# bostoncleek/ergodic_exploration

Hardware: NVIDIA B200
Metric: ergodic control solves/sec (batched) (higher is better)
Workload: dtype f64

## Files before the change

ergodic_exploration_b200/csrc/ergodic_b200.cu:

```cuda
#include "../../include/ergodic_b200.h"

#include <cuda_runtime.h>

#include <algorithm>
#include <atomic>
#include <cmath>
#include <cstdio>
#include <cstdlib>
#include <cstring>
#include <new>
#include <string>
#include <vector>

#include <nvtx3/nvToolsExt.h>

#include "collision_kernels.cuh"
#include "map_target.cuh"
#include "map_target_batch.cuh"
#include "model_kernels.cuh"
#include "peer_gather.cuh"
#include "phik_dmma.cuh"
#include "phik_kernels.cuh"
#include "phik_tma.cuh"
#include "safe_control.cuh"
// ... 299 lines not shown
  cudaFree(p->d_ys);
  cudaFree(p->d_cx);
  cudaFree(p->d_cy);
  cudaFree(p->d_cxp);
  cudaFree(p->d_cxpf);
  cudaFree(p->d_cxt);
  cudaFree(p->d_cxtf);
  cudaFree(p->d_T);
  cudaFree(p->d_parts);
  cudaFree(p->d_phik);
  cudaFree(p->d_sum);
  cudaFree(p->d_phi_stage);
  cudaFree(p->d_done);
  for (double* q : p->w_cxt) cudaFree(q);
  for (double* q : p->w_cxtf) cudaFree(q);
  for (double* q : p->w_cy) cudaFree(q);
  cudaFree(p->d_wraw);
  delete p;
}

eb_status eb_phik_plan_set_stream(eb_phik_plan* p, void* s)
{
  if (!p) return fail(EB_ERR_INVALID_ARGUMENT, "plan is NULL");
  p->stream = static_cast<cudaStream_t>(s);
  return EB_OK;
}

eb_status eb_phik_plan_set_algo(eb_phik_plan* p, int algo)
{
  if (!p) return fail(EB_ERR_INVALID_ARGUMENT, "plan is NULL");
  if (algo < 0 || algo > 5)
    return fail(EB_ERR_INVALID_ARGUMENT, "algo must be 0 (auto), 1 (simple), 2 / 3 (register-streamed DMMA tiles, with / without "
                                         "the mirror fold) or 4 / 5 (TMA-staged DMMA tiles, with / without the mirror fold)");
  if (algo >= 2 && p->nb > 32)
    return fail(EB_ERR_UNSUPPORTED, "num_basis > 32: algo 0 (auto: the TMA tile kernel per block of 32 x 32 orders on large grids, "
                                    "else the simple pair) or 1 (simple pair)");
  if ((algo == 2 || algo == 3) && !eb::phik_dmma_supported(p->nx, p->ny))
    return fail(EB_ERR_UNSUPPORTED, "the register-streamed DMMA phi_k kernel needs nx % 4 == 0 and nx >= 128");
  if (algo >= 4 && (!eb::phik_tma_supported(p->nx, p->ny) || !eb::phik_tma_encoder()))
    return fail(EB_ERR_UNSUPPORTED, "the TMA phi_k kernel needs an even nx >= 64 and a driver with cuTensorMapEncodeTiled");
  p->algo = algo;
  return EB_OK;
}

long long eb_phik_launch_count(const eb_phik_plan* p) { return p ? p->launches : 0; }

eb_status eb_phik_plan_fold(const eb_phik_plan* p, int* fold, double* deviation)
{
  if (!p) return fail(EB_ERR_INVALID_ARGUMENT, "plan is NULL");
  if (fold) *fold = p->fold ? 1 : 0;
  if (deviation) *deviation = p->fold_dev;
  return EB_OK;
}

static eb_status phik_execute(eb_phik_plan* p, const double* phi_dev, double* phik_dev, double* phi_sum_dev,
                              double* raw_dev);

eb_status eb_phik_execute_dev(eb_phik_plan* p, const double* phi_dev, double* phik_dev, double* phi_sum_dev)
{
  if (!p || !phi_dev || !phik_dev) return fail(EB_ERR_INVALID_ARGUMENT, "eb_phik_execute_dev: NULL argument");
  return phik_execute(p, phi_dev, phik_dev, phi_sum_dev, nullptr);
}

eb_status eb_phik_execute_raw_dev(eb_phik_plan* p, const double* phi_dev, double* raw_dev)
{
  if (!p || !phi_dev || !raw_dev) return fail(EB_ERR_INVALID_ARGUMENT, "eb_phik_execute_raw_dev: NULL argument");
  return phik_execute(p, phi_dev, nullptr, nullptr, raw_dev);
}

static eb_status phik_execute(eb_phik_plan* p, const double* phi_dev, double* phik_dev, double* phi_sum_dev,
                              double* raw_dev)
{
  EB_TRACE("eb_phik_execute");
  EB_CUDA(cudaSetDevice(p->device));
  int algo = p->algo;
  if (p->nb > 32 && p->d_wraw && algo != 1 && (reinterpret_cast<uintptr_t>(phi_dev) & 15) == 0)
  {
    const int ld = p->ld, nblk = ld / 32;
    for (int by = 0; by < nblk; by++)
      for (int bx = 0; bx < nblk; bx++)
      {
        const int nbm = std::min(32, p->nb - 32 * std::min(by, bx));
        const eb::PhikTmaOut out{ p->d_done, nbm, nullptr, nullptr, p->d_wraw + 1024 * ((size_t)by * nblk + bx), nullptr };
        const int np = eb::phik_tma_launch(phi_dev, p->nx, p->ny, p->fold ? p->w_cxtf[bx] : p->w_cxt[bx], p->w_cy[by],
                                           p->d_parts, p->max_parts, p->fold, out, p->stream);
        if (np < 0) return fail(EB_ERR_CUDA, std::string("phik_tma_launch (wide): ") + cudaGetErrorString(cudaGetLastError()));
        p->launches += 1;
      }
    eb::phik_assemble_wide<<<(ld * ld + 255) / 256, 256, 0, p->stream>>>(p->d_wraw, p->nb, nblk, ld, phik_dev, phi_sum_dev, raw_dev);
    p->launches += 1;
    EB_CUDA(cudaGetLastError());
    return EB_OK;
  }
  if (p->nb > 32)
  {
    const int ld = p->ld;
    eb::phik_stage1_simple<<<dim3(p->ny, ld / 32), 256, 0, p->stream>>>(phi_dev, p->nx, p->d_cx, ld, p->d_T);
    eb::phik_stage2_simple<<<dim3(p->nb, ld / 32), 256, 0, p->stream>>>(p->d_T, p->ny, p->d_cy, ld, p->d_parts);
    eb::phik_finalize_wide<<<(ld * ld + 255) / 256, 256, 0, p->stream>>>(p->d_parts, p->nb, ld, phik_dev, phi_sum_dev, raw_dev);
    p->launches += 3;
    EB_CUDA(cudaGetLastError());
    return EB_OK;
  }
  const bool big = (long long)p->nx * p->ny >= (1 << 18);
  if (algo == 0)
    algo = (big && eb::phik_tma_supported(p->nx, p->ny) && eb::phik_tma_encoder() && (reinterpret_cast<uintptr_t>(phi_dev) & 15) == 0) ? 4 :
           (big && eb::phik_dmma_supported(p->nx, p->ny))                                                                        ? 2 :
                                                                                                                                   1;
  int nparts = 1;
  const bool fold = (algo == 2 || algo == 4) && p->fold;
  if (algo >= 4)
  {
    const eb::PhikTmaOut out{ p->d_done, p->nb, phik_dev, phi_sum_dev, raw_dev, p->peer };
    nparts = eb::phik_tma_launch(phi_dev, p->nx, p->ny, fold ? p->d_cxtf : p->d_cxt, p->d_cy, p->d_parts, p->max_parts, fold,
                                 out, p->stream);
    if (nparts < 0) return fail(EB_ERR_CUDA, std::string("phik_tma_launch: ") + cudaGetErrorString(cudaGetLastError()));
    p->launches += 1;
    return EB_OK;
  }
  else if (algo >= 2)
  {
    nparts = eb::phik_dmma_launch(phi_dev, p->nx, p->ny, fold ? p->d_cxpf : p->d_cxp, p->d_cy, p->d_parts, p->max_parts,
                                  fold, p->stream);
    if (nparts < 0) return fail(EB_ERR_CUDA, std::string("phik_dmma_launch: ") + cudaGetErrorString(cudaGetLastError()));
    p->launches += 1;
  }
  else
  {
    eb::phik_stage1_simple<<<p->ny, 256, 0, p->stream>>>(phi_dev, p->nx, p->d_cx, eb::kPhikLd, p->d_T);
    eb::phik_stage2_simple<<<32, 256, 0, p->stream>>>(p->d_T, p->ny, p->d_cy, eb::kPhikLd, p->d_parts);
    p->launches += 2;
  }
  eb::phik_finalize<<<1, 1024, 0, p->stream>>>(p->d_parts, nparts, p->nb, fold ? 1 : 0, phik_dev, phi_sum_dev, raw_dev);
  p->launches += 1;
  EB_CUDA(cudaGetLastError());
  return EB_OK;
}

eb_status eb_phik_execute_host(eb_phik_plan* p, const double* phi, double* phik, double* phi_sum)
{
  EB_TRACE("eb_phik_execute_host");
  if (!p || !phi || !phik) return fail(EB_ERR_INVALID_ARGUMENT, "eb_phik_execute_host: NULL argument");
  EB_CUDA(cudaSetDevice(p->device));
  const size_t bytes = sizeof(double) * (size_t)p->nx * p->ny;
  if (!p->d_phi_stage) EB_CUDA(cudaMalloc(&p->d_phi_stage, bytes));
  double* const d_phi = p->d_phi_stage;
  cudaError_t e = cudaMemcpyAsync(d_phi, phi, bytes, cudaMemcpyHostToDevice, p->stream);
  eb_status st = EB_OK;
  if (e == cudaSuccess) st = eb_phik_execute_dev(p, d_phi, p->d_phik, p->d_sum);
  if (e == cudaSuccess && st == EB_OK)
    e = cudaMemcpyAsync(phik, p->d_phik, sizeof(double) * p->nb * p->nb, cudaMemcpyDeviceToHost, p->stream);
  if (e == cudaSuccess && st == EB_OK && phi_sum)
    e = cudaMemcpyAsync(phi_sum, p->d_sum, sizeof(double), cudaMemcpyDeviceToHost, p->stream);
  if (e == cudaSuccess && st == EB_OK) e = cudaStreamSynchronize(p->stream);
  if (st != EB_OK) return st;
  if (e != cudaSuccess) return fail(EB_ERR_CUDA, std::string("eb_phik_execute_host: ") + cudaGetErrorString(e));
  return EB_OK;
}

eb_status eb_phik_from_grid_host(int device, const double* phi, int nx, int ny, double resolution, double lx,
                                 double ly, int nb, double* phik, double* phi_sum)
{
  eb_phik_plan* p = nullptr;
  eb_status st = eb_phik_plan_create(device, nx, ny, resolution, lx, ly, nb, &p);
  if (st != EB_OK) return st;
  st = eb_phik_execute_host(p, phi, phik, phi_sum);
  eb_phik_plan_destroy(p);
  return st;
}

}

struct PeerLaunch
{
  int n_peer = 0;
  double* u0_peer[eb::kMaxPeers] = {};
  unsigned long long* flag_peer[eb::kMaxPeers] = {};
  unsigned long long flag_value = 0;
  unsigned int* done_counter = nullptr;
  const unsigned long long* my_flags = nullptr;
  unsigned long long need = 0;
};

struct eb_controller
{
  eb_config cfg{};
  int N = 0, K = 0, nb = 0, B = 0;
  cudaStream_t stream = nullptr;
  double* d_ut[2] = { nullptr, nullptr };
  int cur = 0;
  double* d_pose = nullptr;
  double* d_hist = nullptr;
  double* d_hist_cos = nullptr;
  long long cos_count = 0;
  double cos_key[4] = { 0.0, 0.0, 0.0, 0.0 };
  long long hist_cap = 0, mem_count = 0;
  double *d_phik = nullptr, *d_lamk = nullptr;
  double *d_u0 = nullptr, *d_metric = nullptr, *d_ck = nullptr, *d_x = nullptr;
  double* d_xt = nullptr;
  double* d_big_scratch = nullptr;
  int big_rows = 0;
  int *d_mem_idx_in = nullptr, *d_mem_idx_out = nullptr;
  int *h_fault = nullptr, *d_fault = nullptr;
  int last_idx_count = 0;
  double lx = 0.0, ly = 0.0;
  double map_pos[2] = { 0.0, 0.0 };
  std::vector<double> gauss_mu, gauss_sigma;
  eb_phik_plan* plan = nullptr;
  double* d_phi_grid = nullptr;
  size_t phi_grid_cells = 0;
  double* d_gauss = nullptr;
  int gauss_cap = 0;
  unsigned long long call = 0;
  long long launches = 0;
  bool have_pose = false;
  bool keep_ck = true;
  const struct PeerLaunch* peer = nullptr;
  bool per_inst = false;
  bool frames_set = false;
  double* d_phik_b = nullptr;
  double* d_frames = nullptr;
  double *d_gmu = nullptr, *d_gsig = nullptr;
  int* d_gcount = nullptr;
  int gmax = 0;
  double* d_bounds = nullptr;
  eb::MapBatchDesc* h_mb_desc = nullptr;
  eb::MapBatchDesc* d_mb_desc = nullptr;
  cudaEvent_t mb_staged = nullptr;
  double* d_mb_slots = nullptr;
  long long mb_slot_units = 0;
  unsigned* d_mb_arrive = nullptr;
  signed char* h_mb_cells = nullptr;
  signed char* d_mb_cells = nullptr;
  size_t mb_cells_bytes = 0;
  int mb_grid = 0;
  struct KeptKey
  {
    unsigned long long grid = 0, map = 0;
    unsigned nx = 0, ny = 0;
    double res = 0.0;
  };
  double* d_kb = nullptr;
  std::vector<int> kb_slot0, kb_cap;
  std::vector<KeptKey> kb_key;
  eb::MapKept* h_mb_kept = nullptr;
  eb::MapKept* d_mb_kept = nullptr;
  int* d_safe_list = nullptr;
  int* d_safe_branch = nullptr;
  double* d_safe_vb = nullptr;
  int safe_grid = 0;

  static double* mapped(const void* host)
  {
    cudaPointerAttributes a{};
    if (cudaPointerGetAttributes(&a, host) != cudaSuccess)
    {
      cudaGetLastError();
      return nullptr;
    }
    return (a.type == cudaMemoryTypeHost && a.devicePointer) ? static_cast<double*>(a.devicePointer) : nullptr;
  }
};

inline int zero_copy_max_batch()
{
  static const int v = [] {
    const char* e = std::getenv("EB_ZEROCOPY_MAX_BATCH");
    return e ? std::atoi(e) : 16384;
  }();
  return v;
}

inline bool replay_cos_cache()
{
  static const bool v = [] {
    const char* e = std::getenv("EB_REPLAY_COS");
    return !e || std::atoi(e) != 0;
  }();
  return v;
}

namespace
{
template <int MODEL, int NB, bool V2, bool PER_INST = false>
struct SolveLaunch
{
  static constexpr int kWide = []() constexpr {
    if constexpr (V2)
      return eb::Solve2Cfg<NB>::kWideWarps;
    else
      return eb::SolveCfg<NB>::kWideWarps;
  }();
  static size_t smem(int N, int warps = eb::kSolveWarps)
  {
    if constexpr (V2)
      return eb::solve2_smem_bytes<NB>(N, warps);
    else
      return eb::solve_smem_bytes(eb::SolveCfg<NB>::kTabDoubles, eb::SolveCfg<NB>::kFields, (N + 31) / 32, warps);
  }
  template <int WARPS>
  static cudaError_t launch_w(const eb::SolveParams& p, cudaStream_t s)
  {
    const size_t bytes = smem(p.N, WARPS);
    static size_t configured[64] = {};
    int dev = 0;
    cudaGetDevice(&dev);
    auto kernel = [] {
      if constexpr (V2)
        return eb::solve_kernel2<MODEL, NB, WARPS, PER_INST>;
      else
        return eb::solve_kernel<MODEL, NB, WARPS, PER_INST>;
    }();
    if (bytes > configured[dev & 63])
    {
      cudaError_t e = cudaFuncSetAttribute(kernel, cudaFuncAttributeMaxDynamicSharedMemorySize, (int)bytes);
      if (e != cudaSuccess) return e;
      configured[dev & 63] = bytes;
    }
    const int grid = (p.B + WARPS - 1) / WARPS;
    cudaLaunchConfig_t cfg = {};
    cfg.gridDim = dim3((unsigned)grid);
    cfg.blockDim = dim3((unsigned)(WARPS * 32));
    cfg.dynamicSmemBytes = bytes;
    cfg.stream = s;
    cudaLaunchAttribute at[1];
    at[0].id = cudaLaunchAttributeProgrammaticStreamSerialization;
    at[0].val.programmaticStreamSerializationAllowed = 1;
    cfg.attrs = at;
    cfg.numAttrs = 1;
    return cudaLaunchKernelEx(&cfg, kernel, p);
  }
  static cudaError_t launch(const eb::SolveParams& p, cudaStream_t s)
  {
    static const int sms = [] {
      int dev = 0, n = 148;
      cudaGetDevice(&dev);
      cudaDeviceGetAttribute(&n, cudaDevAttrMultiProcessorCount, dev);
      return n;
    }();
    static const bool wide_ok = [] {
      const char* e = std::getenv("EB_SOLVE_WIDE");
      return !e || std::atoi(e) != 0;
    }();
    if (wide_ok && p.n_peer == 0 && p.B <= sms * kWide && p.B > sms * eb::kSolveWarps && smem(p.N, kWide) + 2048 <= wide_limit())
      return launch_w<kWide>(p, s);
    return launch_w<eb::kSolveWarps>(p, s);
  }
  static size_t wide_limit()
  {
    static const size_t lim = [] {
      int dev = 0, v = 0;
      cudaGetDevice(&dev);
      cudaDeviceGetAttribute(&v, cudaDevAttrMaxSharedMemoryPerBlockOptin, dev);
      return (size_t)v;
    }();
    return lim;
  }
};

template <int MODEL, bool PER_INST>
cudaError_t launch_solve_big(const eb::SolveParams& p, cudaStream_t s)
{
  const size_t bytes = eb::solve_big_smem_bytes(p.nb, p.N);
  static size_t configured[64] = {};
  int dev = 0;
  cudaGetDevice(&dev);
  if (bytes > configured[dev & 63])
  {
    cudaError_t e = cudaFuncSetAttribute(eb::solve_kernel_big<MODEL, PER_INST>, cudaFuncAttributeMaxDynamicSharedMemorySize, (int)bytes);
    if (e != cudaSuccess) return e;
    configured[dev & 63] = bytes;
  }
  if (!p.big_scratch || p.big_rows < 1) return cudaErrorInvalidValue;
  const int grid = std::min(p.B, p.big_rows);
  eb::solve_kernel_big<MODEL, PER_INST><<<grid, eb::kBigThreads, bytes, s>>>(p, p.big_scratch);
  return cudaGetLastError();
}

int solve_big_resident(int nb, int N)
{
  const size_t bytes = eb::solve_big_smem_bytes(nb, N);
  int dev = 0, sms = 148, per_sm = 0;
  cudaGetDevice(&dev);
  cudaDeviceGetAttribute(&sms, cudaDevAttrMultiProcessorCount, dev);
  if (cudaFuncSetAttribute(eb::solve_kernel_big<0>, cudaFuncAttributeMaxDynamicSharedMemorySize, (int)bytes) != cudaSuccess ||
      cudaOccupancyMaxActiveBlocksPerMultiprocessor(&per_sm, eb::solve_kernel_big<0>, eb::kBigThreads, bytes) != cudaSuccess)
  {
    cudaGetLastError();
    per_sm = 1;
  }
  return sms * std::max(1, per_sm);
}

template <int MODEL, bool PER_INST, class F>
auto with_solve_launch(int nb, F&& f)
{
  if (nb <= 8) return f(SolveLaunch<MODEL, 8, false, PER_INST>{});
  if (nb <= 10) return f(SolveLaunch<MODEL, 10, false, PER_INST>{});
  if (nb <= 12) return f(SolveLaunch<MODEL, 12, false, PER_INST>{});
  if (nb <= 16) return f(SolveLaunch<MODEL, 16, true, PER_INST>{});
  if (nb <= 20) return f(SolveLaunch<MODEL, 20, true, PER_INST>{});
  if (nb <= 24) return f(SolveLaunch<MODEL, 24, true, PER_INST>{});
  return f(SolveLaunch<MODEL, 32, false, PER_INST>{});
}

template <int MODEL, bool PER_INST>
cudaError_t launch_solve_m(const eb::SolveParams& p, cudaStream_t s)
{
  if (p.nb > 32) return launch_solve_big<MODEL, PER_INST>(p, s);
  return with_solve_launch<MODEL, PER_INST>(p.nb, [&](auto L) { return decltype(L)::launch(p, s); });
}

size_t solve_smem_for(int nb, int N)
{
  if (nb > 32) return eb::solve_big_smem_bytes(nb, N);
  return with_solve_launch<0, false>(nb, [&](auto L) { return decltype(L)::smem(N); });
}

cudaError_t launch_solve(const eb::SolveParams& p, int model, cudaStream_t s, bool per_inst)
{
  if (per_inst)
    return model == EB_MODEL_OMNI ? launch_solve_m<eb::kModelOmni, true>(p, s) :
                                    launch_solve_m<eb::kModelSimpleCart, true>(p, s);
  return model == EB_MODEL_OMNI ? launch_solve_m<eb::kModelOmni, false>(p, s) :
                                  launch_solve_m<eb::kModelSimpleCart, false>(p, s);
}

eb_status ensure_hist(eb_controller* c, long long need)
{
  if (need <= c->hist_cap) return EB_OK;
  long long cap = std::max<long long>(c->hist_cap ? 2 * c->hist_cap : 128, need);
  {
    size_t free_b = 0, total_b = 0;
    const size_t full = sizeof(double) * (replay_cos_cache() ? 5 : 3) * (size_t)c->B * (size_t)c->cfg.buffer_size;
    if (cudaMemGetInfo(&free_b, &total_b) == cudaSuccess && full <= free_b / 8) cap = std::max<long long>(cap, c->cfg.buffer_size);
  }
  cap = std::min<long long>(cap, std::max<long long>((long long)c->cfg.buffer_size, need));
  double* nh = nullptr;
  EB_CUDA(cudaMalloc(&nh, sizeof(double) * 3 * (size_t)c->B * (size_t)cap));
  if (c->mem_count > 0)
    EB_CUDA(cudaMemcpyAsync(nh, c->d_hist, sizeof(double) * 3 * (size_t)c->B * (size_t)c->mem_count,
                            cudaMemcpyDeviceToDevice, c->stream));
  EB_CUDA(cudaStreamSynchronize(c->stream));
  cudaFree(c->d_hist);
  c->d_hist = nh;
  c->hist_cap = cap;
  if (replay_cos_cache() && c->per_inst)
  {
    double* nc = nullptr;
    EB_CUDA(cudaMalloc(&nc, sizeof(double) * 2 * (size_t)c->B * (size_t)cap));
    if (c->mem_count > 0 && c->d_hist_cos)
    {
      EB_CUDA(cudaMemcpyAsync(nc, c->d_hist_cos, sizeof(double) * 2 * (size_t)c->B * (size_t)c->mem_count,
                              cudaMemcpyDeviceToDevice, c->stream));
      EB_CUDA(cudaStreamSynchronize(c->stream));
    }
    cudaFree(c->d_hist_cos);
    c->d_hist_cos = nc;
  }
  else if (replay_cos_cache())
  {
    cudaFree(c->d_hist_cos);
    c->d_hist_cos = nullptr;
    c->cos_count = 0;
    EB_CUDA(cudaMalloc(&c->d_hist_cos, sizeof(double) * 2 * (size_t)c->B * (size_t)cap));
  }
  return EB_OK;
}

eb_status ensure_hist_cos(eb_controller* c)
{
  if (!c->d_hist_cos || c->mem_count == 0) return EB_OK;
  const double key[4] = { c->map_pos[0], c->map_pos[1], 1.0 / c->lx, 1.0 / c->ly };
  if (std::memcmp(key, c->cos_key, sizeof(key)) != 0)
  {
    std::memcpy(c->cos_key, key, sizeof(key));
    c->cos_count = 0;
  }
  if (c->cos_count < c->mem_count)
  {
    const long long n = (c->mem_count - c->cos_count) * (long long)c->B;
    const size_t off = (size_t)c->cos_count * (size_t)c->B;
    eb::hist_cos_kernel<<<(unsigned)((n + 255) / 256), 256, 0, c->stream>>>(c->d_hist + 3 * off, c->d_hist_cos + 2 * off, n,
                                                                            key[0], key[1], key[2], key[3]);
    EB_CUDA(cudaGetLastError());
    c->launches += 1;
    c->cos_count = c->mem_count;
  }
  return EB_OK;
}

eb_status check_fault(eb_controller* c)
{
  EB_CUDA(cudaStreamSynchronize(c->stream));
  const int f = *static_cast<volatile int*>(c->h_fault);
  if (f)
  {
    *c->h_fault = 0;
    if (f & 2)
      return fail(EB_ERR_OUT_OF_RANGE, "replay-buffer sample index outside [0, stored states)");
    if (f & 4) return fail(EB_ERR_CUDA, "control(): non-finite state or control signal (NaN / Inf guard)");
    if (f & eb::kFaultTarget)
      return fail(EB_ERR_INVALID_ARGUMENT, "per-instance target: an instance's map extent changed but it has no "
                                           "Gaussians (eb_set_target_gaussians_batch), or its extent is not positive");
    return fail(EB_ERR_INVALID_ARGUMENT, "Invalid twist y-velocity must be 0.");
  }
  return EB_OK;
}

eb_status refuse_per_inst(const char* call)
{
  return fail(EB_ERR_INVALID_ARGUMENT, std::string(call) + ": the controller holds one target per instance (it has "
                                                           "taken an eb_*_batch target call); use the _batch calls");
}

eb_status ensure_per_inst(eb_controller* c)
{
  if (c->per_inst) return EB_OK;
  EB_CUDA(cudaSetDevice(c->cfg.device));
  const size_t pb = sizeof(double) * (size_t)c->K * c->B, fb = sizeof(double) * eb::kFrDoubles * (size_t)c->B;
  EB_CUDA(cudaMalloc(&c->d_phik_b, pb));
  EB_CUDA(cudaMalloc(&c->d_frames, fb));
  EB_CUDA(cudaMalloc(&c->d_gcount, sizeof(int) * (size_t)c->B));
  EB_CUDA(cudaMalloc(&c->d_bounds, sizeof(double) * 4 * (size_t)c->B));
  EB_CUDA(cudaMemsetAsync(c->d_phik_b, 0, pb, c->stream));
  EB_CUDA(cudaMemsetAsync(c->d_frames, 0, fb, c->stream));
  EB_CUDA(cudaMemsetAsync(c->d_gcount, 0, sizeof(int) * (size_t)c->B, c->stream));
  c->per_inst = true;
  return EB_OK;
}

eb_status target_batch(eb_controller* c, const double* bounds_dev, const double* extent_dev, int* rebuilt_dev)
{
  eb::TargetBatchParams tp{};
  tp.B = c->B;
  tp.nb = c->nb;
  tp.max_n = c->gmax;
  tp.res = c->cfg.resolution;
  tp.bounds = bounds_dev;
  tp.extent = extent_dev;
  tp.counts = c->d_gcount;
  tp.mu = c->d_gmu;
  tp.sigma = c->d_gsig;
  tp.frames = c->d_frames;
  tp.phik = c->d_phik_b;
  tp.rebuilt = rebuilt_dev;
  tp.hist = c->d_hist;
  tp.hist_cos = c->d_hist_cos;
  tp.mem_count = c->d_hist_cos ? c->mem_count : 0;
  tp.fault = c->d_fault;
  eb::target_batch_kernel<<<c->B, eb::kTbThreads, sizeof(double) * 6 * (size_t)c->gmax, c->stream>>>(tp);
  EB_CUDA(cudaGetLastError());
  c->launches += 1;
  c->frames_set = true;
  return EB_OK;
}
}

extern "C" {

eb_status eb_create(const eb_config* cfg, eb_controller** out)
{
  if (!out) return fail(EB_ERR_INVALID_ARGUMENT, "eb_create: out is NULL");
  *out = nullptr;
  if (!cfg) return fail(EB_ERR_INVALID_ARGUMENT, "eb_create: cfg is NULL");
  if (cfg->model != EB_MODEL_SIMPLE_CART && cfg->model != EB_MODEL_OMNI)
    return fail(EB_ERR_INVALID_ARGUMENT, "eb_create: unknown model (only the 3-twist models SimpleCart and Omni "
                                         "can be driven by ErgodicControl)");
  if (cfg->batch < 1) return fail(EB_ERR_INVALID_ARGUMENT, "eb_create: batch must be >= 1");
  if (cfg->num_basis < 1 || cfg->num_basis > EB_MAX_NUM_BASIS)
    return fail(EB_ERR_INVALID_ARGUMENT, "eb_create: num_basis must be in 1.." + std::to_string(EB_MAX_NUM_BASIS));
  if (!(cfg->dt != 0.0) || !std::isfinite(cfg->horizon / cfg->dt))
    return fail(EB_ERR_INVALID_ARGUMENT, "eb_create: dt must be non-zero and finite");
  const unsigned steps = static_cast<unsigned>(std::abs(cfg->horizon / cfg->dt));
  if (steps == 1)
    return fail(EB_ERR_INVALID_ARGUMENT,
                "Need at least two steps in forward simulation. Increase the horizon or decrease the time step.");
  if (steps == 0) return fail(EB_ERR_INVALID_ARGUMENT, "eb_create: horizon / dt gives zero steps");
  if (steps > 4096) return fail(EB_ERR_UNSUPPORTED, "eb_create: more than 4096 horizon steps is not supported");
  if (eb_device_count() < 1) return fail(EB_ERR_NO_DEVICE, "no CUDA device is visible; there is no CPU fallback");
  EB_CUDA(cudaSetDevice(cfg->device));
  {
    int optin = 0;
    EB_CUDA(cudaDeviceGetAttribute(&optin, cudaDevAttrMaxSharedMemoryPerBlockOptin, cfg->device));
    const size_t need = solve_smem_for(static_cast<int>(cfg->num_basis), static_cast<int>(steps));
    if (need > static_cast<size_t>(optin))
      return fail(EB_ERR_UNSUPPORTED, "eb_create: a horizon of " + std::to_string(steps) + " steps with num_basis " +
                                          std::to_string(cfg->num_basis) + " needs " + std::to_string(need) +
                                          " bytes of shared memory per block; the device allows " + std::to_string(optin));
  }

  eb_controller* c = new (std::nothrow) eb_controller();
  if (!c) return fail(EB_ERR_CUDA, "out of host memory");
  c->cfg = *cfg;
  c->N = (int)steps;
  c->nb = (int)cfg->num_basis;
  c->K = c->nb * c->nb;
  c->B = cfg->batch;
  const size_t utb = sizeof(double) * 3 * (size_t)c->N * c->B;
  auto cleanup = [&](eb_status st) {
    eb_destroy(c);
    return st;
  };
#define EB_CUDA_C(expr)                                                                      \
  do                                                                                         \
  {                                                                                          \
    cudaError_t e__ = (expr);                                                                \
    if (e__ != cudaSuccess)                                                                  \
      return cleanup(fail(EB_ERR_CUDA, std::string(#expr) + ": " + cudaGetErrorString(e__))); \
  } while (0)
  EB_CUDA_C(cudaMalloc(&c->d_ut[0], utb));
  EB_CUDA_C(cudaMalloc(&c->d_ut[1], utb));
  EB_CUDA_C(cudaMemset(c->d_ut[0], 0, utb));
  EB_CUDA_C(cudaMemset(c->d_ut[1], 0, utb));
  EB_CUDA_C(cudaMalloc(&c->d_pose, sizeof(double) * 3 * c->B));
  EB_CUDA_C(cudaMemset(c->d_pose, 0, sizeof(double) * 3 * c->B));
  EB_CUDA_C(cudaMalloc(&c->d_x, sizeof(double) * 3 * c->B));
  EB_CUDA_C(cudaMalloc(&c->d_u0, sizeof(double) * 3 * c->B));
  EB_CUDA_C(cudaMalloc(&c->d_metric, sizeof(double) * c->B));
  EB_CUDA_C(cudaMalloc(&c->d_ck, sizeof(double) * (size_t)c->K * c->B));
// ... 3310 lines not shown
```

ergodic_exploration_b200/csrc/solve_kernel.cuh:

```cuda
#pragma once

#include "common.cuh"

namespace eb
{
constexpr int kModelSimpleCart = 0;
constexpr int kModelOmni = 1;
constexpr int kSolveWarps = 4;
constexpr int kMaxPeers = 8;
constexpr int kPeerBuffers = 4;
constexpr int kTabSlots = 16;
constexpr int kTabStride = 20;

#ifdef EB_PHASE_TIMING
constexpr int kPhaseSlots = 16;
__device__ long long g_phase[65536 * kPhaseSlots];
#define EB_PHASE(idx)                                                                      \
  do                                                                                       \
  {                                                                                        \
    if (lane == 0 && inst < 65536) g_phase[inst * kPhaseSlots + (idx)] = clock64();        \
  } while (0)
#else
#define EB_PHASE(idx) do { } while (0)
#endif

#ifdef EB_DEBUG_DUMP
__device__ double g_dbg[4096 * 16];
#endif

#ifndef EB_ABL
#define EB_ABL 0
#endif
__device__ __forceinline__ void abl_xor(double& d0, double a, double b)
{
  d0 = __hiloint2double(__double2hiint(d0), __double2loint(d0) ^ __double2loint(a) ^ __double2hiint(b));
}
__device__ __forceinline__ void dmma_ck(double& d0, double& d1, double a, double b)
{
#if EB_ABL & 1
  abl_xor(d0, a, b);
#else
  dmma884(d0, d1, a, b);
#endif
}
__device__ __forceinline__ void dmma_gr(double& d0, double& d1, double a, double b)
{
#if EB_ABL & 2
  abl_xor(d0, a, b);
#else
  dmma884(d0, d1, a, b);
#endif
}

struct SolveParams
{
  int B, N, M, nb;
  int mem_count, batch_size, idx_mode;
  double dt, lx, ly, inv_lx, inv_ly, ax, by, xmin, ymin, w;
  double Rinv[9], umin[3], umax[3], bw, beps;
  unsigned long long seed, call;
  const double* x;
  double* pose_out;
  const double* ut_in;
  double* ut_out;
  const double* hist;
  const double* hist_cos;
  const int* mem_idx;
  int* mem_idx_out;
  const double* phik;
  const double* lamk;
  double* u0;
  double* metric;
  double* ck;
  int* fault;
  int n_peer;
  double* u0_peer[kMaxPeers];
  unsigned long long* flag_peer[kMaxPeers];
  unsigned long long flag_value;
  unsigned int* done_counter;
  const unsigned long long* my_flags;
  unsigned long long need;
  double* big_scratch;
  int big_rows;
  const double* frames;
};

enum FrameField
{
  kFrXmin,
  kFrYmin,
  kFrLx,
  kFrLy,
  kFrInvLx,
  kFrInvLy,
  kFrAx,
  kFrBy,
  kFrDoubles
};

template <bool PER_INST, int F>
__device__ __forceinline__ double frame(const SolveParams& p, const int inst)
{
  if constexpr (PER_INST)
    return __ldg(p.frames + (size_t)inst * kFrDoubles + F);
  else if constexpr (F == kFrXmin)
    return p.xmin;
  else if constexpr (F == kFrYmin)
    return p.ymin;
  else if constexpr (F == kFrLx)
    return p.lx;
  else if constexpr (F == kFrLy)
    return p.ly;
  else if constexpr (F == kFrInvLx)
    return p.inv_lx;
  else if constexpr (F == kFrInvLy)
    return p.inv_ly;
  else if constexpr (F == kFrAx)
    return p.ax;
  else
    return p.by;
}

template <bool PER_INST>
__device__ __forceinline__ double phik_at(const SolveParams& p, const int inst, const int K, const int k)
{
  if constexpr (PER_INST)
    return __ldg(p.phik + (size_t)inst * K + k);
  else
    return __ldg(p.phik + k);
}

__device__ __forceinline__ void publish_first_twist(const SolveParams& p, const int inst, const int lane, const double (&un)[3])
{
  const double a0 = __shfl_sync(kFull, un[0], 0), a1 = __shfl_sync(kFull, un[1], 0), a2 = __shfl_sync(kFull, un[2], 0);
  const double mine = lane == 0 ? a0 : (lane == 1 ? a1 : a2);
  if (lane < 3) p.u0[(size_t)inst * 3 + lane] = mine;
  if (p.n_peer > 0)
  {
    if (lane < p.n_peer)
      while (*(const volatile unsigned long long*)(p.my_flags + lane) < p.need) __nanosleep(100);
    __syncwarp();
    if (lane < 3)
    {
#pragma unroll
      for (int q = 0; q < kMaxPeers; q++)
        if (q < p.n_peer) p.u0_peer[q][(size_t)inst * 3 + lane] = mine;
    }
    __threadfence();
    __syncwarp();
    if (lane == 0)
    {
      const unsigned int prev = atomicAdd(p.done_counter, 1u);
      if (prev == (unsigned int)p.B - 1u)
      {
        *p.done_counter = 0u;
        __threadfence_system();
#pragma unroll
        for (int q = 0; q < kMaxPeers; q++)
          if (q < p.n_peer) *(volatile unsigned long long*)p.flag_peer[q] = p.flag_value;
      }
    }
  }
}

template <int WARPS>
struct WideIo
{
  static constexpr bool kOn = WARPS > kSolveWarps;
  double x[kOn ? 3 * WARPS : 1];
  double u0[kOn ? 3 * WARPS : 1];
  unsigned int arrived;
};

template <int WARPS>
__device__ __forceinline__ void wide_io_load(WideIo<WARPS>& io, const SolveParams& p)
{
  const int first = blockIdx.x * WARPS;
  const int cnt = min(WARPS, p.B - first);
  if ((int)threadIdx.x < 3 * cnt) io.x[threadIdx.x] = p.x[(size_t)first * 3 + threadIdx.x];
  if (threadIdx.x == 0) io.arrived = 0u;
  __syncthreads();
}

template <int WARPS>
__device__ __forceinline__ void wide_io_store(WideIo<WARPS>& io, const SolveParams& p, const int lane, const int warp,
                                              const double (&un)[3])
{
  const double a0 = __shfl_sync(kFull, un[0], 0), a1 = __shfl_sync(kFull, un[1], 0), a2 = __shfl_sync(kFull, un[2], 0);
  if (lane < 3) io.u0[3 * warp + lane] = lane == 0 ? a0 : (lane == 1 ? a1 : a2);
  const int first = blockIdx.x * WARPS;
  const int cnt = min(WARPS, p.B - first);
  __syncwarp();
  unsigned int last = 0u;
  if (lane == 0)
  {
    __threadfence_block();
    last = atomicAdd(&io.arrived, 1u) == (unsigned int)(cnt - 1) ? 1u : 0u;
    __threadfence_block();
  }
  if (__shfl_sync(kFull, last, 0))
    for (int i = lane; i < 3 * cnt; i += 32) p.u0[(size_t)first * 3 + i] = io.u0[i];
}

__device__ __forceinline__ void grid_dependency_wait()
{
  asm volatile("griddepcontrol.wait;" ::: "memory");
  asm volatile("griddepcontrol.launch_dependents;" ::: "memory");
}

template <int MODEL>
__device__ __forceinline__ void model_f(double u0, double u1, double c, double s, double& fx, double& fy)
{
  if (MODEL == kModelOmni)
  {
    fx = u0 * c - u1 * s;
    fy = u0 * s + u1 * c;
  }
  else
  {
    fx = u0 * c;
    fy = u0 * s;
  }
}

struct RolloutCarry
{
  double x, y, th, cth, sth;
};

template <int MODEL>
__device__ __forceinline__ void rollout_round(const double dt, const bool valid, const int lane, const double u0,
                                              const double u1, const double u2, RolloutCarry& cy, double& xo,
                                              double& yo, double& tho, double& ce, double& se)
{
  const double dth = valid ? (dt / 6.0) * (((u2 + 2.0 * u2) + 2.0 * u2) + u2) : 0.0;
  const double inc = warp_scan_incl(dth, lane);
  double exc = __shfl_up_sync(kFull, inc, 1);
  if (lane == 0) exc = 0.0;
  const double th_before = cy.th + exc;
  tho = cy.th + inc;
  const double thm = th_before + dt * (0.5 * u2);
  double sm, cm;
  fast_sincos(tho, &se, &ce);
  fast_sincos(thm, &sm, &cm);
  double cb = __shfl_up_sync(kFull, ce, 1), sb = __shfl_up_sync(kFull, se, 1);
  if (lane == 0)
  {
    cb = cy.cth;
    sb = cy.sth;
  }
  double k1x, k1y, k2x, k2y, k4x, k4y;
  model_f<MODEL>(u0, u1, cb, sb, k1x, k1y);
  model_f<MODEL>(u0, u1, cm, sm, k2x, k2y);
  model_f<MODEL>(u0, u1, ce, se, k4x, k4y);
  const double dx = valid ? (dt / 6.0) * (((k1x + 2.0 * k2x) + 2.0 * k2x) + k4x) : 0.0;
  const double dy = valid ? (dt / 6.0) * (((k1y + 2.0 * k2y) + 2.0 * k2y) + k4y) : 0.0;
  xo = cy.x + warp_scan_incl(dx, lane);
  yo = cy.y + warp_scan_incl(dy, lane);
  cy.x = __shfl_sync(kFull, xo, 31);
  cy.y = __shfl_sync(kFull, yo, 31);
  cy.th = __shfl_sync(kFull, tho, 31);
  cy.cth = __shfl_sync(kFull, ce, 31);
  cy.sth = __shfl_sync(kFull, se, 31);
}

template <int NB>
__device__ __forceinline__ void coeff_chunk(double* __restrict__ tabx, const int lane, const bool valid,
                                            const int nvalid, const double c1x, const double c1y,
                                            double (&acc)[(NB + 7) / 8][(NB + 7) / 8][2])
{
  constexpr int TILES = (NB + 7) / 8;
  static_assert(NB % 2 == 0, "NB must be even");
  const int g = lane >> 2, q = lane & 3;
  const double* taby = tabx + NB * kTabStride;
  double* const mytab = tabx + (lane >> 4) * (NB * kTabStride) + (lane & 15);
#pragma unroll
  for (int h = 0; h < 2; h++)
  {
    const int left = nvalid - h * kTabSlots;
    if (left <= 0) break;
    {
      const int src = 16 * h + (lane & 15);
      const double sx = __shfl_sync(kFull, c1x, src), sy = __shfl_sync(kFull, c1y, src);
      const bool ok = __shfl_sync(kFull, (int)valid, src) != 0;
      const double v = lane < 16 ? sx : sy;
      const double m = fma(4.0 * v, v, -2.0);
      double em = ok ? fma(2.0 * v, v, -1.0) : 0.0, ek = ok ? 1.0 : 0.0;
      double om = ok ? v : 0.0, ok1 = om;
      __syncwarp();
#if EB_ABL & 4
      mytab[0] = ek + ok1 + em * m;
#else
#pragma unroll
      for (int k = 0; k < NB; k += 2)
      {
        mytab[k * kTabStride] = ek;
        mytab[(k + 1) * kTabStride] = ok1;
        const double en = fma(m, ek, -em), on = fma(m, ok1, -om);
        em = ek;
        ek = en;
        om = ok1;
        ok1 = on;
      }
#endif
    }
    __syncwarp();
    const int ksteps = (min(left, kTabSlots) + 3) >> 2;
    for (int s = 0; s < ksteps; s++)
    {
      double a[TILES], b[TILES];
#pragma unroll
      for (int t = 0; t < TILES; t++)
      {
        const int k = 8 * t + g;
        const bool in = (TILES * 8 == NB) || (k < NB);
        a[t] = in ? taby[k * kTabStride + 4 * s + q] : 0.0;
        b[t] = in ? tabx[k * kTabStride + 4 * s + q] : 0.0;
      }
#pragma unroll
      for (int ti = 0; ti < TILES; ti++)
#pragma unroll
        for (int tj = 0; tj < TILES; tj++) dmma_ck(acc[ti][tj][0], acc[ti][tj][1], a[ti], b[tj]);
    }
  }
}

template <int NB>
struct SolveCfg
{
  static constexpr bool kRecompute = NB >= 16;
  static constexpr int kFields = kRecompute ? 4 : 8;
  static constexpr int kSPitch = NB;
  static constexpr int kTabDoubles = 2 * NB * kTabStride;
  static constexpr int kBlock = NB <= 12 ? NB : 8;
  static constexpr int kMinBlocks = NB <= 10 ? 7 : NB <= 12 ? 6 : 4;
  static constexpr int kWideWarps = NB <= 10 ? 28 : NB <= 12 ? 24 : 16;
  static_assert(NB <= 12 || NB == 32, "num_basis 13..24 run solve_kernel2");
  static_assert(NB % kBlock == 0, "kx blocks must tile NB");
};

inline size_t solve_smem_bytes(int tab_doubles, int fields, int rounds, int warps = kSolveWarps)
{
  return sizeof(double) * warps * (size_t)(tab_doubles + fields * 32 * rounds);
}

template <int MODEL, int NB, int WARPS = kSolveWarps, bool PER_INST = false>
__global__ void __launch_bounds__(WARPS * 32, WARPS == kSolveWarps ? SolveCfg<NB>::kMinBlocks : 1) solve_kernel(const SolveParams p)
{
  using Cfg = SolveCfg<NB>;
  constexpr int TILES = (NB + 7) / 8;
  constexpr int KB = Cfg::kBlock;
  extern __shared__ double smem[];
  const int lane = threadIdx.x & 31, warp = threadIdx.x >> 5;
  const int rounds = (p.N + 31) >> 5;
  const int npad = rounds * 32;
  const int nb = p.nb, K = nb * nb;

  const int inst = blockIdx.x * WARPS + warp;
  __shared__ WideIo<WARPS> wio;
  grid_dependency_wait();
  double e_u0 = 0.0, e_u1 = 0.0, e_u2 = 0.0;
  if (inst < p.B && lane + 1 < p.N)
  {
    const double* e_in = p.ut_in + ((size_t)inst * p.N + lane + 1) * 3;
    e_u0 = e_in[0];
    e_u1 = e_in[1];
    e_u2 = e_in[2];
  }
  if constexpr (WideIo<WARPS>::kOn) wide_io_load(wio, p);
  if (inst >= p.B) return;
#if EB_ABL & 128
  if (lane < 3) p.u0[(size_t)inst * 3 + lane] = 0.0;
  return;
#endif
  EB_PHASE(0);

  double* tabx = smem + warp * (Cfg::kTabDoubles + Cfg::kFields * npad);
  double* rec = tabx + Cfg::kTabDoubles;
  double* Ssm = tabx;

  double acc[TILES][TILES][2];
#pragma unroll
  for (int i = 0; i < TILES; i++)
#pragma unroll
    for (int j = 0; j < TILES; j++) acc[i][j][0] = acc[i][j][1] = 0.0;

  for (int base = 0; base < p.M; base += 32)
  {
    const int j = base + lane;
    const bool valid = j < p.M;
    double c1x = 1.0, c1y = 1.0;
    if (valid)
    {
      long long idx = j;
      if (p.idx_mode == 1)
        idx = p.mem_idx[(size_t)inst * p.batch_size + j];
      else if (p.idx_mode == 2)
      {
        const uint64_t r = mix64(mix64(p.seed + p.call * 0xD1B54A32D192ED03ull) ^
                                 ((uint64_t)inst * 0x9E3779B97F4A7C15ull + (uint64_t)j));
        idx = (long long)__umul64hi(r, (uint64_t)p.mem_count);
      }
      if ((unsigned long long)idx >= (unsigned long long)p.mem_count)
      {
        atomicOr(p.fault, 2);
        idx = 0;
      }
      if (p.idx_mode != 0 && p.mem_idx_out) p.mem_idx_out[(size_t)inst * p.batch_size + j] = (int)idx;
      if (p.hist_cos)
      {
        const double2 hc = *reinterpret_cast<const double2*>(p.hist_cos + ((size_t)idx * p.B + inst) * 2);
        c1x = hc.x;
        c1y = hc.y;
      }
      else
      {
        const double* h = p.hist + ((size_t)idx * p.B + inst) * 3;
        const double xf = h[0] - frame<PER_INST, kFrXmin>(p, inst), yf = h[1] - frame<PER_INST, kFrYmin>(p, inst);
        c1x = fast_cospi(xf * frame<PER_INST, kFrInvLx>(p, inst));
        c1y = fast_cospi(yf * frame<PER_INST, kFrInvLy>(p, inst));
      }
    }
    const int nvalid = min(32, p.M - base);
    coeff_chunk<NB>(tabx, lane, valid, nvalid, c1x, c1y, acc);
  }

  EB_PHASE(1);
  const double* ut_in = p.ut_in + (size_t)inst * p.N * 3;
  double* ut_out = p.ut_out + (size_t)inst * p.N * 3;
  RolloutCarry cy;
  {
    double xv = 0.0;
    if constexpr (WideIo<WARPS>::kOn)
      xv = lane < 3 ? wio.x[3 * warp + lane] : 0.0;
    else
      xv = lane < 3 ? p.x[(size_t)inst * 3 + lane] : 0.0;
    if (p.pose_out && lane < 3) p.pose_out[(size_t)inst * 3 + lane] = xv;
    cy.x = __shfl_sync(kFull, xv, 0);
    cy.y = __shfl_sync(kFull, xv, 1);
    cy.th = __shfl_sync(kFull, xv, 2);
    fast_sincos(cy.th, &cy.sth, &cy.cth);
  }
  for (int r = 0; r < rounds; r++)
  {
    const int i = r * 32 + lane;
    const bool valid = i < p.N;
    double u0 = 0.0, u1 = 0.0, u2 = 0.0;
    if (r == 0)
    {
      u0 = e_u0;
      u1 = e_u1;
      u2 = e_u2;
    }
    else if (i + 1 < p.N)
    {
      u0 = ut_in[(i + 1) * 3 + 0];
      u1 = ut_in[(i + 1) * 3 + 1];
      u2 = ut_in[(i + 1) * 3 + 2];
    }
    if (MODEL == kModelSimpleCart && !(fabs(u1 - 0.0) < 1.0e-12)) atomicOr(p.fault, 1);
    double xo, yo, tho, ce, se;
    rollout_round<MODEL>(p.dt, valid, lane, u0, u1, u2, cy, xo, yo, tho, ce, se);
    const double xf = xo - frame<PER_INST, kFrXmin>(p, inst), yf = yo - frame<PER_INST, kFrYmin>(p, inst);
    rec[0 * npad + i] = ce;
    rec[1 * npad + i] = se;
    rec[2 * npad + i] = xf;
    rec[3 * npad + i] = yf;
    double ca, cb;
    if (Cfg::kRecompute)
    {
      ca = fast_cospi(xf * frame<PER_INST, kFrInvLx>(p, inst));
      cb = fast_cospi(yf * frame<PER_INST, kFrInvLy>(p, inst));
    }
    else
    {
      double sa, sb;
      fast_sincospi(xf * frame<PER_INST, kFrInvLx>(p, inst), &sa, &ca);
      fast_sincospi(yf * frame<PER_INST, kFrInvLy>(p, inst), &sb, &cb);
      rec[4 * npad + i] = ca;
      rec[5 * npad + i] = sa;
      rec[6 * npad + i] = cb;
      rec[7 * npad + i] = sb;
    }
    const int nvalid = min(32, p.N - r * 32);
    if (r < 2) EB_PHASE(2 + 2 * r);
    coeff_chunk<NB>(tabx, lane, valid, nvalid, ca, cb, acc);
    if (r < 2) EB_PHASE(3 + 2 * r);
  }

  __syncwarp();
  {
    const int g = lane >> 2, q = lane & 3;
    const double inv_t = 1.0 / (double)(p.M + p.N);
    double metric = 0.0;
#pragma unroll
    for (int ti = 0; ti < TILES; ti++)
#pragma unroll
      for (int tj = 0; tj < TILES; tj++)
#pragma unroll
        for (int e = 0; e < 2; e++)
        {
          const int ky = 8 * ti + g, kx = 8 * tj + 2 * q + e;
          double s = 0.0;
          if (ky < nb && kx < nb)
          {
            const int k = ky * nb + kx;
            const double c = __dmul_rn(inv_t, acc[ti][tj][e]);
            const double d = __dsub_rn(c, phik_at<PER_INST>(p, inst, K, k));
            s = __ldg(p.lamk + k) * d;
            metric += s * d;
            if (p.ck) p.ck[(size_t)inst * K + k] = c;
          }
          if (ky < NB && kx < NB) Ssm[ky * Cfg::kSPitch + kx] = s;
        }
    if (p.metric)
    {
      metric = warp_sum(metric);
      if (lane == 0) p.metric[inst] = metric;
    }
  }
  __syncwarp();
  EB_PHASE(6);

  double r0c = 0.0, r1c = 0.0, r2c = 0.0;
  for (int r = rounds - 1; r >= 0; r--)
  {
    const int i = r * 32 + lane;
    const bool valid = i < p.N;
    const double ce = rec[0 * npad + i], se = rec[1 * npad + i];
    const double xf = rec[2 * npad + i], yf = rec[3 * npad + i];
    double u0 = 0.0, u1 = 0.0;
    if (i + 1 < p.N)
    {
      u0 = ut_in[(i + 1) * 3 + 0];
      u1 = ut_in[(i + 1) * 3 + 1];
    }
    double ca, sa, cb, sb;
    if (Cfg::kRecompute)
    {
      fast_sincospi(xf * frame<PER_INST, kFrInvLx>(p, inst), &sa, &ca);
      fast_sincospi(yf * frame<PER_INST, kFrInvLy>(p, inst), &sb, &cb);
    }
    else
    {
      ca = rec[4 * npad + i];
      sa = rec[5 * npad + i];
      cb = rec[6 * npad + i];
      sb = rec[7 * npad + i];
    }
    double ex = 0.0, ey = 0.0;
    double xcm = ca, xck = 1.0, xsm = -sa, xsk = 0.0;
    const double xt2 = 2.0 * ca, yt2 = 2.0 * cb;
#pragma unroll
    for (int kb = 0; kb < NB; kb += KB)
    {
      double cx[KB], asx[KB];
#pragma unroll
      for (int j = 0; j < KB; j++)
      {
        cx[j] = xck;
        asx[j] = ((double)(kb + j) * frame<PER_INST, kFrAx>(p, inst)) * xsk;
        const double cn = xt2 * xck - xcm, sn = xt2 * xsk - xsm;
        xcm = xck;
        xck = cn;
        xsm = xsk;
        xsk = sn;
      }
      double cm = cb, ck = 1.0, sm = -sb, sk = 0.0;
#pragma unroll 2
      for (int ky = 0; ky < NB; ky++)
      {
        double rx0 = 0.0, rx1 = 0.0, ry0 = 0.0, ry1 = 0.0;
        const double* srow = Ssm + ky * Cfg::kSPitch + kb;
#pragma unroll
        for (int j = 0; j < KB; j += 2)
        {
          const double2 s2 = *reinterpret_cast<const double2*>(srow + j);
          rx0 = fma(s2.x, asx[j], rx0);
          rx1 = fma(s2.y, asx[j + 1], rx1);
          ry0 = fma(s2.x, cx[j], ry0);
          ry1 = fma(s2.y, cx[j + 1], ry1);
        }
        ex = fma(ck, rx0 + rx1, ex);
        ey = fma(((double)ky * frame<PER_INST, kFrBy>(p, inst)) * sk, ry0 + ry1, ey);
        const double cn = yt2 * ck - cm, sn = yt2 * sk - sm;
        cm = ck;
        ck = cn;
        sm = sk;
        sk = sn;
      }
    }
    ex = -ex * p.w;
    ey = -ey * p.w;
    if (rounds - 1 - r < 2) EB_PHASE(7 + 2 * (rounds - 1 - r));
#ifdef EB_DEBUG_DUMP
    if (inst == 0 && i < 4096)
    {
      double* d = g_dbg + i * 16;
      d[0] = ex; d[1] = ey; d[2] = ca; d[3] = sa; d[4] = cb; d[5] = sb; d[6] = ce; d[7] = se; d[8] = xf; d[9] = yf;
      d[10] = Ssm[lane % (NB * NB)];
    }
#endif

    double bx = 0.0, byv = 0.0;
    bx += 2.0 * (double)(xf > frame<PER_INST, kFrLx>(p, inst) - p.beps) * (xf - (frame<PER_INST, kFrLx>(p, inst) - p.beps));
    byv += 2.0 * (double)(yf > frame<PER_INST, kFrLy>(p, inst) - p.beps) * (yf - (frame<PER_INST, kFrLy>(p, inst) - p.beps));
    bx += 2.0 * (double)(xf < p.beps) * (xf - p.beps);
    byv += 2.0 * (double)(yf < p.beps) * (yf - p.beps);
    bx *= p.bw;
    byv *= p.bw;
    const double k0 = valid ? (-ex - bx) : 0.0;
    const double k1 = valid ? (-ey - byv) : 0.0;
    const double inc0 = -(p.dt / 6.0 * (((k0 + 2.0 * k0) + 2.0 * k0) + k0));
    const double inc1 = -(p.dt / 6.0 * (((k1 + 2.0 * k1) + 2.0 * k1) + k1));
    const double suf0 = warp_scan_incl_rev(inc0, lane);
    const double suf1 = warp_scan_incl_rev(inc1, lane);
    double exc0 = __shfl_down_sync(kFull, suf0, 1), exc1 = __shfl_down_sync(kFull, suf1, 1);
    if (lane == 31) exc0 = exc1 = 0.0;
    const double r0p = r0c + exc0, r1p = r1c + exc1;
    const double r0 = r0c + suf0, r1 = r1c + suf1;
    double a02, a12;
    if (MODEL == kModelOmni)
    {
      a02 = -u0 * se - u1 * ce;
      a12 = u0 * ce - u1 * se;
    }
    else
    {
      a02 = -u0 * se;
      a12 = u0 * ce;
    }
    const double k1_2 = -(a02 * r0p + a12 * r1p);
    const double r0s = r0p - p.dt * (0.5 * k0), r1s = r1p - p.dt * (0.5 * k1);
    const double k2_2 = -(a02 * r0s + a12 * r1s);
    const double r0e = r0p - p.dt * k0, r1e = r1p - p.dt * k1;
    const double k4_2 = -(a02 * r0e + a12 * r1e);
    const double inc2 = valid ? -(p.dt / 6.0 * (((k1_2 + 2.0 * k2_2) + 2.0 * k2_2) + k4_2)) : 0.0;
    const double r2 = r2c + warp_scan_incl_rev(inc2, lane);
    r0c = __shfl_sync(kFull, r0, 0);
    r1c = __shfl_sync(kFull, r1, 0);
    r2c = __shfl_sync(kFull, r2, 0);
    double bt0, bt1;
    if (MODEL == kModelOmni)
    {
      bt0 = ce * r0 + se * r1;
      bt1 = -se * r0 + ce * r1;
    }
    else
    {
      bt0 = ce * r0 + se * r1;
      bt1 = 0.0;
    }
    double un[3];
    bool finite = true;
#pragma unroll
    for (int c = 0; c < 3; c++)
    {
      const double v = -((p.Rinv[c + 0] * bt0 + p.Rinv[c + 3] * bt1) + p.Rinv[c + 6] * r2);
      finite &= fabs(v) <= 1.7976931348623157e308;
      un[c] = clampd(v, p.umin[c], p.umax[c]);
      if (valid) ut_out[i * 3 + c] = un[c];
    }
    if (valid && !finite) atomicOr(p.fault, 4);
    if (r == 0)
    {
      if constexpr (WideIo<WARPS>::kOn)
        wide_io_store(wio, p, lane, warp, un);
      else
        publish_first_twist(p, inst, lane, un);
    }
    if (rounds - 1 - r < 2) EB_PHASE(8 + 2 * (rounds - 1 - r));
  }
  EB_PHASE(11);
#ifdef EB_PHASE_TIMING
  if (lane == 0 && inst < 65536)
  {
    unsigned smid;
    asm volatile("mov.u32 %0, %%smid;" : "=r"(smid));
    g_phase[inst * kPhaseSlots + 15] = smid;
  }
#endif
}

__global__ void __launch_bounds__(256) hist_cos_kernel(const double* __restrict__ hist, double* __restrict__ out, long long n,
                                                       double xmin, double ymin, double inv_lx, double inv_ly)
{
  const long long e = (long long)blockIdx.x * blockDim.x + threadIdx.x;
  if (e >= n) return;
  const double xf = hist[3 * e + 0] - xmin, yf = hist[3 * e + 1] - ymin;
  out[2 * e + 0] = fast_cospi(xf * inv_lx);
  out[2 * e + 1] = fast_cospi(yf * inv_ly);
}
__global__ void __launch_bounds__(256) add_state_kernel(const double* __restrict__ x, double* __restrict__ hist_row,
                                                        double* __restrict__ cos_row, int B, double xmin, double ymin,
                                                        double inv_lx, double inv_ly, const double* __restrict__ frames)
{
  const int i = blockIdx.x * blockDim.x + threadIdx.x;
  if (i >= B) return;
  const double a = x[3 * i + 0], b = x[3 * i + 1], c = x[3 * i + 2];
  hist_row[3 * i + 0] = a;
  hist_row[3 * i + 1] = b;
  hist_row[3 * i + 2] = c;
  if (frames)
  {
    const double* f = frames + (size_t)i * kFrDoubles;
    xmin = f[kFrXmin];
    ymin = f[kFrYmin];
    inv_lx = f[kFrInvLx];
    inv_ly = f[kFrInvLy];
  }
  const double xf = a - xmin, yf = b - ymin;
  cos_row[2 * i + 0] = fast_cospi(xf * inv_lx);
  cos_row[2 * i + 1] = fast_cospi(yf * inv_ly);
}

template <int MODEL>
__global__ void __launch_bounds__(128) rollout_kernel(int B, int N, double dt, const double* __restrict__ pose,
                                                      const double* __restrict__ ut, double* __restrict__ xt,
                                                      int* fault)
{
  const int lane = threadIdx.x & 31;
  const int inst = (blockIdx.x * blockDim.x + threadIdx.x) >> 5;
  if (inst >= B) return;
  const double* u = ut + (size_t)inst * N * 3;
  double* out = xt + (size_t)inst * N * 3;
  RolloutCarry cy;
  cy.x = pose[(size_t)inst * 3 + 0];
  cy.y = pose[(size_t)inst * 3 + 1];
  cy.th = pose[(size_t)inst * 3 + 2];
  fast_sincos(cy.th, &cy.sth, &cy.cth);
  for (int base = 0; base < N; base += 32)
  {
    const int i = base + lane;
    const bool valid = i < N;
    double u0 = 0.0, u1 = 0.0, u2 = 0.0;
    if (valid)
    {
      u0 = u[i * 3 + 0];
      u1 = u[i * 3 + 1];
      u2 = u[i * 3 + 2];
    }
    if (MODEL == kModelSimpleCart && !(fabs(u1 - 0.0) < 1.0e-12)) atomicOr(fault, 1);
    double xo, yo, tho, ce, se;
    rollout_round<MODEL>(dt, valid, lane, u0, u1, u2, cy, xo, yo, tho, ce, se);
    if (valid)
    {
      out[i * 3 + 0] = xo;
      out[i * 3 + 1] = yo;
      out[i * 3 + 2] = normalize_angle_pi(tho);
    }
  }
}
}
```

Baseline: 173.8 million.

## Specialize solve kernel for fixed one or two rounds with hoisted frame scales

Adds a ROUNDS template parameter so horizons of 1–64 steps with num_basis <= 12 run a kernel whose round loops are fully unrolled. In that variant the first of two rounds skips validity checks and shuffles, and the per-term frame scale factors (ax, by) are pulled out of the inner gradient loop and applied once afterwards. The inner FMA chains are also merged into single accumulators. This removes per-iteration multiplies and bounds logic, but changes floating-point summation order, adds kernel instantiations, and lengthens the dependency chain in the inner loop.

```diff
diff --git a/ergodic_exploration_b200/csrc/ergodic_b200.cu b/ergodic_exploration_b200/csrc/ergodic_b200.cu
--- a/ergodic_exploration_b200/csrc/ergodic_b200.cu
+++ b/ergodic_exploration_b200/csrc/ergodic_b200.cu
@@ -625,20 +625,25 @@
   static cudaError_t launch_w(const eb::SolveParams& p, cudaStream_t s)
   {
     const size_t bytes = smem(p.N, WARPS);
-    static size_t configured[64] = {};
+    const int rounds = (!V2 && NB <= 12 && p.N >= 1 && p.N <= 64) ? (p.N + 31) / 32 : 0;
+    static size_t configured[3][64] = {};
     int dev = 0;
     cudaGetDevice(&dev);
-    auto kernel = [] {
+    auto kernel = [rounds] {
       if constexpr (V2)
         return eb::solve_kernel2<MODEL, NB, WARPS, PER_INST>;
+      else if constexpr (NB <= 12)
+        return rounds == 1 ? eb::solve_kernel<MODEL, NB, WARPS, PER_INST, 1> :
+               rounds == 2 ? eb::solve_kernel<MODEL, NB, WARPS, PER_INST, 2> :
+                             eb::solve_kernel<MODEL, NB, WARPS, PER_INST>;
       else
         return eb::solve_kernel<MODEL, NB, WARPS, PER_INST>;
     }();
-    if (bytes > configured[dev & 63])
+    if (bytes > configured[rounds][dev & 63])
     {
       cudaError_t e = cudaFuncSetAttribute(kernel, cudaFuncAttributeMaxDynamicSharedMemorySize, (int)bytes);
       if (e != cudaSuccess) return e;
-      configured[dev & 63] = bytes;
+      configured[rounds][dev & 63] = bytes;
     }
     const int grid = (p.B + WARPS - 1) / WARPS;
     cudaLaunchConfig_t cfg = {};
diff --git a/ergodic_exploration_b200/csrc/solve_kernel.cuh b/ergodic_exploration_b200/csrc/solve_kernel.cuh
--- a/ergodic_exploration_b200/csrc/solve_kernel.cuh
+++ b/ergodic_exploration_b200/csrc/solve_kernel.cuh
@@ -264,7 +264,7 @@
   cy.sth = __shfl_sync(kFull, se, 31);
 }
 
-template <int NB>
+template <int NB, bool FULL = false>
 __device__ __forceinline__ void coeff_chunk(double* __restrict__ tabx, const int lane, const bool valid,
                                             const int nvalid, const double c1x, const double c1y,
                                             double (&acc)[(NB + 7) / 8][(NB + 7) / 8][2])
@@ -277,12 +277,12 @@
 #pragma unroll
   for (int h = 0; h < 2; h++)
   {
-    const int left = nvalid - h * kTabSlots;
+    const int left = (FULL ? 32 : nvalid) - h * kTabSlots;
     if (left <= 0) break;
     {
       const int src = 16 * h + (lane & 15);
       const double sx = __shfl_sync(kFull, c1x, src), sy = __shfl_sync(kFull, c1y, src);
-      const bool ok = __shfl_sync(kFull, (int)valid, src) != 0;
+      const bool ok = FULL || __shfl_sync(kFull, (int)valid, src) != 0;
       const double v = lane < 16 ? sx : sy;
       const double m = fma(4.0 * v, v, -2.0);
       double em = ok ? fma(2.0 * v, v, -1.0) : 0.0, ek = ok ? 1.0 : 0.0;
@@ -344,15 +344,17 @@
   return sizeof(double) * warps * (size_t)(tab_doubles + fields * 32 * rounds);
 }
 
-template <int MODEL, int NB, int WARPS = kSolveWarps, bool PER_INST = false>
+template <int MODEL, int NB, int WARPS = kSolveWarps, bool PER_INST = false, int ROUNDS = 0>
 __global__ void __launch_bounds__(WARPS * 32, WARPS == kSolveWarps ? SolveCfg<NB>::kMinBlocks : 1) solve_kernel(const SolveParams p)
 {
   using Cfg = SolveCfg<NB>;
   constexpr int TILES = (NB + 7) / 8;
   constexpr int KB = Cfg::kBlock;
+  constexpr bool kFixed = ROUNDS > 0;
+  static_assert(ROUNDS >= 0 && ROUNDS <= 2 && (!kFixed || NB <= 12), "fixed rounds: 1 or 2, num_basis <= 12");
   extern __shared__ double smem[];
   const int lane = threadIdx.x & 31, warp = threadIdx.x >> 5;
-  const int rounds = (p.N + 31) >> 5;
+  const int rounds = kFixed ? ROUNDS : (p.N + 31) >> 5;
   const int npad = rounds * 32;
   const int nb = p.nb, K = nb * nb;
 
@@ -360,7 +362,7 @@
   __shared__ WideIo<WARPS> wio;
   grid_dependency_wait();
   double e_u0 = 0.0, e_u1 = 0.0, e_u2 = 0.0;
-  if (inst < p.B && lane + 1 < p.N)
+  if (inst < p.B && (ROUNDS == 2 || lane + 1 < p.N))
   {
     const double* e_in = p.ut_in + ((size_t)inst * p.N + lane + 1) * 3;
     e_u0 = e_in[0];
@@ -441,10 +443,12 @@
     cy.th = __shfl_sync(kFull, xv, 2);
     fast_sincos(cy.th, &cy.sth, &cy.cth);
   }
+#pragma unroll(kFixed ? ROUNDS : 1)
   for (int r = 0; r < rounds; r++)
   {
     const int i = r * 32 + lane;
-    const bool valid = i < p.N;
+    const bool full = ROUNDS == 2 && r == 0;
+    const bool valid = full || i < p.N;
     double u0 = 0.0, u1 = 0.0, u2 = 0.0;
     if (r == 0)
     {
@@ -484,7 +488,10 @@
     }
     const int nvalid = min(32, p.N - r * 32);
     if (r < 2) EB_PHASE(2 + 2 * r);
-    coeff_chunk<NB>(tabx, lane, valid, nvalid, ca, cb, acc);
+    if (full)
+      coeff_chunk<NB, true>(tabx, lane, valid, nvalid, ca, cb, acc);
+    else
+      coeff_chunk<NB>(tabx, lane, valid, nvalid, ca, cb, acc);
     if (r < 2) EB_PHASE(3 + 2 * r);
   }
 
@@ -523,14 +530,16 @@
   EB_PHASE(6);
 
   double r0c = 0.0, r1c = 0.0, r2c = 0.0;
+#pragma unroll(kFixed ? ROUNDS : 1)
   for (int r = rounds - 1; r >= 0; r--)
   {
     const int i = r * 32 + lane;
-    const bool valid = i < p.N;
+    const bool full = ROUNDS == 2 && r == 0;
+    const bool valid = full || i < p.N;
     const double ce = rec[0 * npad + i], se = rec[1 * npad + i];
     const double xf = rec[2 * npad + i], yf = rec[3 * npad + i];
     double u0 = 0.0, u1 = 0.0;
-    if (i + 1 < p.N)
+    if (full || i + 1 < p.N)
     {
       u0 = ut_in[(i + 1) * 3 + 0];
       u1 = ut_in[(i + 1) * 3 + 1];
@@ -559,7 +568,7 @@
       for (int j = 0; j < KB; j++)
       {
         cx[j] = xck;
-        asx[j] = ((double)(kb + j) * frame<PER_INST, kFrAx>(p, inst)) * xsk;
+        asx[j] = kFixed ? (double)(kb + j) * xsk : ((double)(kb + j) * frame<PER_INST, kFrAx>(p, inst)) * xsk;
         const double cn = xt2 * xck - xcm, sn = xt2 * xsk - xsm;
         xcm = xck;
         xck = cn;
@@ -576,19 +585,32 @@
         for (int j = 0; j < KB; j += 2)
         {
           const double2 s2 = *reinterpret_cast<const double2*>(srow + j);
-          rx0 = fma(s2.x, asx[j], rx0);
-          rx1 = fma(s2.y, asx[j + 1], rx1);
-          ry0 = fma(s2.x, cx[j], ry0);
-          ry1 = fma(s2.y, cx[j + 1], ry1);
+          if constexpr (kFixed)
+          {
+            rx0 = fma(s2.y, asx[j + 1], fma(s2.x, asx[j], rx0));
+            ry0 = fma(s2.y, cx[j + 1], fma(s2.x, cx[j], ry0));
+          }
+          else
+          {
+            rx0 = fma(s2.x, asx[j], rx0);
+            rx1 = fma(s2.y, asx[j + 1], rx1);
+            ry0 = fma(s2.x, cx[j], ry0);
+            ry1 = fma(s2.y, cx[j + 1], ry1);
+          }
         }
-        ex = fma(ck, rx0 + rx1, ex);
-        ey = fma(((double)ky * frame<PER_INST, kFrBy>(p, inst)) * sk, ry0 + ry1, ey);
+        ex = fma(ck, kFixed ? rx0 : rx0 + rx1, ex);
+        ey = fma((kFixed ? (double)ky : (double)ky * frame<PER_INST, kFrBy>(p, inst)) * sk, kFixed ? ry0 : ry0 + ry1, ey);
         const double cn = yt2 * ck - cm, sn = yt2 * sk - sm;
         cm = ck;
         ck = cn;
         sm = sk;
         sk = sn;
       }
+    }
+    if constexpr (kFixed)
+    {
+      ex *= frame<PER_INST, kFrAx>(p, inst);
+      ey *= frame<PER_INST, kFrBy>(p, inst);
     }
     ex = -ex * p.w;
     ey = -ey * p.w;
```

Result: faster. 180.2 million (median of 6 runs) (+3.7%).
